# FudanCVL/SynFMC

Measured on AMD Instinct MI355X. Metric: denoising steps/sec, 16x320x512 bf16 U-Net+CMC+OMC, higher is better.
Workload: dtype bf16; 1 GPU; 16x320x512 clip, CFG batch 2, full-width 3D U-Net (1.39B params, random init) + Camera Adapter (CMC) + Object Motion Control (OMC) features, DDIM step; configs/obj.yaml shapes; 1 clip per GPU; frames=16, height=320, width=512, hip_graph=True, fp8_temporal_attention=False, parallelism=dp1 (independent clips, no collective)

## Files before the change

synfmc_amd/csrc/gemm_conv.hip:

```cpp
#include <stdlib.h>

#include <algorithm>
#include <type_traits>

#include "common.h"

namespace {

constexpr int BK_MAX = 64;

struct GemmParams {
    const bf16_t* a; const bf16_t* w; const bf16_t* bias; const bf16_t* temb; const bf16_t* res; bf16_t* out;
    const bf16_t* res2;
    int64_t M; int N, K;
    int64_t lda, ldres, ldo;
    int img_h, img_w, cin, hw;
    int64_t temb_ld; int temb_div;
    const bf16_t* a2; int64_t lda2; int ksplit;
    int ups;
    float alpha;
    int tiles_m, tiles_n;
    int regepi;
    int tap_outer;
    int group_m;
// ... 605 lines not shown
#pragma unroll
                    for (int k = 0; k < 8; ++k) a[k] = (a[k] + ba[k]) * gelu_erf(g[k] + bg[k]);
                    Vec8<bf16_t>::store(P.out + m * P.ldo + no, a);
                }
            }
        }
    }
    if (!SK) break;
    if (sk_partial) {
        asm volatile("s_waitcnt vmcnt(0)" ::: "memory");
        __syncthreads();
        if (tid == 0)
            __hip_atomic_store(P.sk_flags + blockIdx.x, 1, __ATOMIC_RELAXED, __HIP_MEMORY_SCOPE_AGENT);
    } else if (sk_np > 0) {
        __syncthreads();
        if (tid == 0)
            for (int j = 1; j <= sk_np; ++j)
                __hip_atomic_store(P.sk_flags + (blockIdx.x - 8 * j), 0, __ATOMIC_RELAXED, __HIP_MEMORY_SCOPE_AGENT);
    }
    __syncthreads();
    }
}

template <int MODE, int EPI, int PF, int ROLE>
__global__ __launch_bounds__(512, 2)
void gemm8_kernel(const GemmParams P) {
    constexpr int BM = 256, BN = 256, BK = 64, NT = 512;
    constexpr int STAGE_ELEMS = (BM + BN) * BK;
    constexpr int VMW = 2 * (PF - 2);
    static_assert(PF >= 3 && PF <= 6, "prefetch distance (half-tiles)");
    extern __shared__ __attribute__((aligned(16))) unsigned char smem_raw[];
    bf16_t* smem = reinterpret_cast<bf16_t*>(smem_raw);
    const int wave = __builtin_amdgcn_readfirstlane(threadIdx.x >> 6);
    const int wr = wave >> 2, wc = wave & 3;

    const int nkt = P.K / BK;
    constexpr bool SK = ROLE == 1 || ROLE == 3;
    int64_t sk_it = 0, sk_end = 0, sk_gbase = 0, sk_I = 0;
    int sk_r = 0, sk_per = 1, sk_first = 0;
    int lk_u = 0;
    if (SK && P.sk_lock) {
        lk_u = (int)(blockIdx.x & 7) * (P.sk >> 3) + (int)(blockIdx.x >> 3);
    } else if (SK) {
        const int T = P.tiles_m * P.tiles_n - P.sk_t0, x = blockIdx.x & 7, q = blockIdx.x >> 3;
        sk_per = P.sk >> 3;
        const int tg0 = (int)((int64_t)T * x / 8), tg1 = (int)((int64_t)T * (x + 1) / 8);
        sk_gbase = (int64_t)tg0 * nkt;
        sk_I = (int64_t)(tg1 - tg0) * nkt;
        sk_r = sk_per - 1 - q;
// ... 95 lines not shown
#pragma unroll
                        for (int gq = 0; gq < 4; ++gq) {
                            const int quad = (wave * 8 + ni * 4 + mi) * 4 + gq;
                            t[gq] = __builtin_amdgcn_raw_buffer_load_b128(rsP, (int)(((int64_t)slot * (BM * BN / 4) + quad * 64 + lane) * 16), 0, 0);
                        }
#pragma unroll
                        for (int gq = 0; gq < 4; ++gq) {
                            union { u32x4 u; f32x4 f; } c;
                            c.u = t[gq];
                            acc[ni][mi][4 * gq] += c.f[0]; acc[ni][mi][4 * gq + 1] += c.f[1];
                            acc[ni][mi][4 * gq + 2] += c.f[2]; acc[ni][mi][4 * gq + 3] += c.f[3];
                        }
                    }
            }
        }
    }
    const int64_t m0 = (int64_t)tile_m * BM;
    const int n0 = tile_n * BN;

    constexpr unsigned OOB = 0x80000000u;
    const __amdgpu_buffer_rsrc_t rsA = __builtin_amdgcn_make_buffer_rsrc((void*)P.a, 0, (int)P.a_bytes, 0x00020000);
    const __amdgpu_buffer_rsrc_t rsW = __builtin_amdgcn_make_buffer_rsrc((void*)P.w, 0, (int)((int64_t)P.N * P.K * 2), 0x00020000);
    unsigned a_vo[4];
    unsigned a_ok[4];
    unsigned w_vo[4];
    int a_lds[4], w_lds[4];
#pragma unroll
    for (int e = 0; e < 4; ++e) {
        const int late = e >> 1, u = 2 * wave + (e & 1);
        const int rowa = (u >> 3) * 128 + late * 64 + (u & 7) * 8;
        a_lds[e] = rowa * BK;
        const int lr = rowa + prow;
        const int sc = swz<BK>(lr, pch);
        const int64_t m = m0 + lr;
        const bool ok = m < P.M;
        a_ok[e] = 0;
        if (MODE == 0) {
            a_vo[e] = ok ? (unsigned)((m * P.lda + sc * 8) * 2) : OOB;
        } else {
            const int64_t mm = ok ? m : 0;
            const int pix = (int)(mm % P.hw);
            const int py = pix / P.img_w, px = pix - py * P.img_w;
            const int64_t img = mm / P.hw;
            if (P.ups == 1) {
                a_vo[e] = ok ? (unsigned)((img * (int64_t)(P.hw >> 2) * P.cin + sc * 8) * 2) : OOB;
                a_ok[e] = ((unsigned)py << 16) | (unsigned)px;
            } else {
                unsigned mask = 0;
                for (int t = 0; t < 9; ++t) {
                    const int dy = t / 3 - 1, dx = t % 3 - 1;
                    const bool in = P.ups == 2 ? (2 * py + dy >= 0 && 2 * px + dx >= 0)
                                               : ((unsigned)(py + dy) < (unsigned)P.img_h && (unsigned)(px + dx) < (unsigned)P.img_w);
                    mask |= (unsigned)in << t;
                }
                a_ok[e] = ok ? mask : 0u;
                if (P.ups == 2) a_vo[e] = (unsigned)(((img * (int64_t)(P.hw << 2) + (int64_t)(2 * py) * (2 * P.img_w) + 2 * px) * P.cin + sc * 8) * 2);
                else a_vo[e] = (unsigned)((mm * P.cin + sc * 8) * 2);
            }
        }
        const int roww = (u >> 2) * 64 + late * 32 + (u & 3) * 8;
        w_lds[e] = (BM + roww) * BK;
// ... 22 lines not shown
            seek(kt0);
        } else if (MODE == 1) {
            if (P.tap_outer) {
                it_ci0 += BK;
                if (it_ci0 == P.cin) { it_ci0 = 0; ++it_tap; }
            } else if (++it_tap == 9) {
                it_tap = 0;
                it_ci0 += BK;
            }
        }
    };
    auto dma = [&](const __amdgpu_buffer_rsrc_t& rs, unsigned voff, int soff, bf16_t* lds) {
        __builtin_amdgcn_raw_ptr_buffer_load_lds(rs, (__attribute__((address_space(3))) void*)lds, 16, (int)voff, soff, 0, 0);
    };
    auto issue = [&](int q) {
        bf16_t* stage = smem + it_buf * STAGE_ELEMS;
        if (q == 1 || q == 2) {
            const int e0 = (q - 1) * 2;
            const int soff = (MODE == 1 ? it_tap * P.cin + it_ci0 : it_kt * BK) * 2;
#pragma unroll
            for (int i = 0; i < 2; ++i) dma(rsW, w_vo[e0 + i], soff, stage + w_lds[e0 + i]);
        } else {
            const int e0 = q == 0 ? 0 : 2;
            if (MODE == 0) {
#pragma unroll
                for (int i = 0; i < 2; ++i) dma(rsA, a_vo[e0 + i], it_kt * BK * 2, stage + a_lds[e0 + i]);
            } else {
                const int dy = (it_tap >= 3) + (it_tap >= 6) - 1, dx = it_tap - 3 * (dy + 1) - 1;
#pragma unroll
                for (int i = 0; i < 2; ++i) {
                    const int e = e0 + i;
                    unsigned vo;
                    if (P.ups == 1) {
                        const int py = (int)(a_ok[e] >> 16) + dy, px = (int)(a_ok[e] & 0xffffu) + dx;
                        const bool in = (unsigned)py < (unsigned)P.img_h && (unsigned)px < (unsigned)P.img_w;
                        vo = a_vo[e] + (unsigned)(((py >> 1) * (P.img_w >> 1) + (px >> 1)) * P.cin * 2);
                        if (!in || a_vo[e] == OOB) vo = OOB;
                    } else {
                        const int shift = (P.ups == 2 ? (dy * 2 * P.img_w + dx) : (dy * P.img_w + dx)) * P.cin * 2;
                        vo = ((a_ok[e] >> it_tap) & 1u) ? a_vo[e] + (unsigned)shift : OOB;
                    }
                    dma(rsA, vo, it_ci0 * 2, stage + a_lds[e]);
                }
            }
        }
        if (q == 3) advance();
    };
// ... 296 lines not shown
}
__device__ __forceinline__ void gn_tile_finish(const GemmParams& P, float* red, int64_t m0, int n0, int cpg, int tid, float s, float ss) {
    const int GT = 320 / cpg, RP = 512 / GT;
    red[2 * tid] = s;
    red[2 * tid + 1] = ss;
    __syncthreads();
    if (tid < GT) {
        float a = 0.f, b = 0.f;
        for (int k = 0; k < RP; ++k) { a += red[2 * (tid + k * GT)]; b += red[2 * (tid + k * GT) + 1]; }
        const int64_t img = m0 / P.gn_hw;
        const int nsplit = P.gn_hw / 160, sp = (int)((m0 - img * P.gn_hw) / 160);
        float* dst = P.gn_part + ((img * nsplit + sp) * 32 + (n0 / cpg + tid)) * 2;
        dst[0] = a;
        dst[1] = b;
    }
}

__device__ __forceinline__ void lane32_swap(float& lo_keeps, float& hi_keeps) {
    auto r = __builtin_amdgcn_permlane32_swap(__float_as_uint(lo_keeps), __float_as_uint(hi_keeps), false, false);
    lo_keeps = __uint_as_float(r[0]);
    hi_keeps = __uint_as_float(r[1]);
}

template <int MODE, int EPI>
__global__ __launch_bounds__(512, 2)
void gemm160_kernel(const GemmParams P) {
    constexpr int BM = 160, BN = 320, BK = 32, NT = 512, NBUF = 5;
    constexpr int SUB_ELEMS = (BM + BN) * BK;
    extern __shared__ __attribute__((aligned(16))) unsigned char smem_raw[];
    bf16_t* smem = reinterpret_cast<bf16_t*>(smem_raw);
    const int wave = __builtin_amdgcn_readfirstlane(threadIdx.x >> 6);
    const int wr = wave >> 2, wc = wave & 3;
    const int tid = threadIdx.x, lane = tid & 63;
    const int l15 = lane & 15, kq = lane >> 4;
    const int prow = lane >> 2, pch = lane & 3;
    const int psrc = pch ^ (3 * ((prow >> 3) & 1));

    int nks = P.K / BK, ks0 = 0;
    int tile_m, tile_n;
    const int split = P.split_k > 1 ? (int)(blockIdx.x % P.split_k) : 0;
    {
        const int total = P.tiles_m * P.tiles_n;
        int lin = blockIdx.x;
        if (P.split_k > 1) {
            lin = blockIdx.x / P.split_k;
            const int per = ((nks + P.split_k - 1) / P.split_k + 1) & ~1;
            ks0 = split * per;
            nks = max(0, min(nks, ks0 + per) - ks0);
        } else {
            const int id = blockIdx.x, q = total >> 3, r = total & 7, x = id & 7;
            lin = (x < r ? x * (q + 1) : r * (q + 1) + (x - r) * q) + (id >> 3);
        }
        lin_to_tile(lin, P, tile_m, tile_n);
    }
    const int64_t m0 = (int64_t)tile_m * BM;
    const int n0 = tile_n * BN;

    constexpr unsigned OOB = 0x80000000u;
    const __amdgpu_buffer_rsrc_t rsA = __builtin_amdgcn_make_buffer_rsrc((void*)P.a, 0, (int)P.a_bytes, 0x00020000);
    const __amdgpu_buffer_rsrc_t rsW = __builtin_amdgcn_make_buffer_rsrc((void*)P.w, 0, (int)((int64_t)P.N * P.K * 2), 0x00020000);
    unsigned e_vo[4], e_ok[4];
    int e_lds[4];
#pragma unroll
    for (int e = 0; e < 4; ++e) {
        const int i = 4 * wave + e;
        e_vo[e] = OOB; e_ok[e] = 0; e_lds[e] = NBUF * SUB_ELEMS;
        if (i < 20) {
            const int lw = 16 * i + prow, n = n0 + lw;
            e_lds[e] = (BM + 16 * i) * BK;
            e_vo[e] = n >= P.N ? OOB : (P.w_blocked ? (unsigned)((((int64_t)tile_n * (P.K / BK)) * (BN * BK) + lw * BK + psrc * 8) * 2)
                                                     : (unsigned)(((int64_t)n * P.K + psrc * 8) * 2));
        } else if (i < 30) {
            const int lr = 16 * (i - 20) + prow;
            e_lds[e] = 16 * (i - 20) * BK;
            const int64_t m = m0 + lr;
            const bool ok = m < P.M;
            if (MODE == 0) {
                e_vo[e] = ok ? (P.a_blocked ? (unsigned)((((int64_t)tile_m * (P.K / BK)) * (BM * BK) + lr * BK + psrc * 8) * 2)
                                            : (unsigned)((m * P.lda + psrc * 8) * 2)) : OOB;
            } else {
                const int64_t mm = ok ? m : 0;
                const int pix = (int)(mm % P.hw);
                const int py = pix / P.img_w, px = pix - py * P.img_w;
                const int64_t img = mm / P.hw;
                if (P.ups == 1) {
                    e_vo[e] = ok ? (unsigned)((img * (int64_t)(P.hw >> 2) * P.cin + psrc * 8) * 2) : OOB;
                    e_ok[e] = ((unsigned)py << 16) | (unsigned)px;
                } else {
                    unsigned mask = 0;
                    for (int t = 0; t < 9; ++t) {
                        const int dy = t / 3 - 1, dx = t % 3 - 1;
                        const bool in = P.ups == 2 ? (2 * py + dy >= 0 && 2 * px + dx >= 0)
                                                   : ((unsigned)(py + dy) < (unsigned)P.img_h && (unsigned)(px + dx) < (unsigned)P.img_w);
                        mask |= (unsigned)in << t;
                    }
                    e_ok[e] = ok ? mask : 0u;
                    if (P.ups == 2) e_vo[e] = (unsigned)(((img * (int64_t)(P.hw << 2) + (int64_t)(2 * py) * (2 * P.img_w) + 2 * px) * P.cin + psrc * 8) * 2);
                    else e_vo[e] = (unsigned)((mm * P.cin + psrc * 8) * 2);
                }
            }
        }
    }
// ... 13 lines not shown
            seek0();
        } else if (MODE == 1) {
            if (++it_half == 2) {
                it_half = 0;
                if (++it_tap == 9) { it_tap = 0; it_ci0 += 64; }
            }
        }
    };
    auto dma = [&](const __amdgpu_buffer_rsrc_t& rs, unsigned voff, int soff, bf16_t* lds) {
        __builtin_amdgcn_raw_ptr_buffer_load_lds(rs, (__attribute__((address_space(3))) void*)lds, 16, (int)voff, soff, 0, 0);
    };
    auto issue = [&]() {
        bf16_t* stage = smem + it_buf * SUB_ELEMS;
        const int kw = P.w_blocked ? it_s * (BN * BK * 2)
                                   : (MODE == 1 ? it_tap * P.cin + it_ci0 + it_half * 32 : it_s * BK) * 2;
        if (w_wave) {
#pragma unroll
            for (int e = 0; e < 4; ++e) dma(rsW, e_vo[e], kw, stage + e_lds[e]);
        } else {
            const int dy = (it_tap >= 3) + (it_tap >= 6) - 1, dx = it_tap - 3 * (dy + 1) - 1;
#pragma unroll
            for (int e = 0; e < 4; ++e) {
                bf16_t* dst = e_lds[e] == NBUF * SUB_ELEMS ? smem + NBUF * SUB_ELEMS : stage + e_lds[e];
                if (MODE == 0) {
                    dma(rsA, e_vo[e], P.a_blocked ? it_s * (BM * BK * 2) : it_s * BK * 2, dst);
                } else {
                    unsigned vo;
                    if (P.ups == 1) {
                        const int py = (int)(e_ok[e] >> 16) + dy, px = (int)(e_ok[e] & 0xffffu) + dx;
                        const bool in = (unsigned)py < (unsigned)P.img_h && (unsigned)px < (unsigned)P.img_w;
                        vo = e_vo[e] + (unsigned)(((py >> 1) * (P.img_w >> 1) + (px >> 1)) * P.cin * 2);
                        if (!in || e_vo[e] == OOB) vo = OOB;
                    } else {
                        const int shift = (P.ups == 2 ? (dy * 2 * P.img_w + dx) : (dy * P.img_w + dx)) * P.cin * 2;
                        vo = ((e_ok[e] >> it_tap) & 1u) ? e_vo[e] + (unsigned)shift : OOB;
                    }
                    dma(rsA, vo, (it_ci0 + it_half * 32) * 2, dst);
                }
            }
        }
        advance();
    };
    (void)a_first;

    f32x4 acc[5][5];
    bf16x8 wf[5], af[5];
    const int frag_off = l15 * BK + (kq ^ (3 * ((l15 >> 3) & 1))) * 8;
// ... 880 lines not shown
            P.sk_lock_len = L;
            fmc_launch<sk_main>(dim3((unsigned)g), dim3(512), lds, st, P);
            if constexpr (EPI == 0) hipLaunchKernelGGL((sk_finish_kernel<MODE>), dim3((unsigned)tiles * 64), dim3(256), 0, st, P);
            else fmc_launch<sk_finish>(dim3((unsigned)tiles), dim3(512), lds, st, P);
            return;
        }
        P.sk_lock = 0;
    }
    if (P.sk) {
        const int64_t iters = (int64_t)tiles * (P.K / 64);
        const int g = fmc_cu_count() & ~7;
        const int maxseg = (tiles + g - 1) / g + 2;
        const int64_t need = (int64_t)g * maxseg * 256 * 256 * (int64_t)sizeof(float) + 4096;
        if (g >= 8 && iters >= 2 * (int64_t)g && P.sk_ws_bytes >= need && need < ((int64_t)1 << 31)) {
            P.sk = g;
            P.sk_maxseg = maxseg;
            P.sk_whole = 0;
            fmc_launch<sk_main>(dim3((unsigned)g), dim3(512), lds, st, P);
            fmc_launch<sk_finish>(dim3((unsigned)tiles), dim3(512), lds, st, P);
            return;
        }
        P.sk = 0;
    }
    fmc_launch<plain>(dim3((unsigned)tiles), dim3(512), lds, st, P);
}

constexpr int K320_K = 320;
template <int MI, int NI> constexpr int k320_stage_chunks() { return ((32 * MI * ((160 * NI + 8) / 8) + 63) / 64) * 64; }
template <int MI, int NI> constexpr size_t k320_lds() {
    return (size_t)2 * 32 * MI * K320_K * 2 + (size_t)k320_stage_chunks<MI, NI>() * 16 + 160 * NI * sizeof(float);
}

template <int MI, int NI, bool HAS_RES>
__global__ __launch_bounds__(320, (MI * NI == 1 ? 3 : (MI * NI == 2 ? 2 : 1))) void gemm_k320_kernel(const GemmParams P) {
    constexpr int K = K320_K, KS = K / 16, BM = 32 * MI, BN = 160 * NI, OP = BN + 8, CPR = K / 8, OCPR = OP / 8, WC = 32 * NI;
    constexpr int A_ELEMS = BM * K, A_PIECES = BM * CPR / 64, ST_PIECES = k320_stage_chunks<MI, NI>() / 64;
    constexpr int A_PPW = (A_PIECES + 4) / 5, ST_PPW = (ST_PIECES + 4) / 5;
    extern __shared__ __attribute__((aligned(16))) unsigned char smem_raw[];
    bf16_t* Abuf = reinterpret_cast<bf16_t*>(smem_raw);
    bf16_t* Os = Abuf + 2 * A_ELEMS;
    float* bias_s = reinterpret_cast<float*>(Os + k320_stage_chunks<MI, NI>() * 8);
    const int tid = threadIdx.x, lane = tid & 63, wave = __builtin_amdgcn_readfirstlane(tid >> 6);
    const int l31 = lane & 31, half = lane >> 5;
    const int n0 = blockIdx.y * BN;
    const int ntiles = (int)(P.M / BM);

// ... 136 lines not shown
    const int bn = (gemm_k320_cfg() % 10 == 1) ? 160 : 320;
    return !P.f32io && P.hw <= 1 && P.K == K320_K && P.N % bn == 0 && P.M % 64 == 0 && !P.a2 && !P.res2 && P.split_k == 1 && !P.sk && !P.temb &&
           ((P.M - 1) * P.lda + P.K) * 2 < ((int64_t)1 << 31) && (!P.res || ((P.M - 1) * P.ldres + P.N) * 2 < ((int64_t)1 << 31));
}

template <int MI, int NI>
void launch_gemm_k320_c(GemmParams& P, hipStream_t st) {
    const size_t lds = k320_lds<MI, NI>();
    const int per_cu = MI * NI == 1 ? 3 : (MI * NI == 2 ? 2 : 1);
    const int tiles = (int)(P.M / (32 * MI)), slots = fmc_cu_count() * per_cu;
    dim3 grid((unsigned)(tiles < slots ? tiles : slots), (unsigned)(P.N / (160 * NI)));
    if (P.res) fmc_launch<gemm_k320_kernel<MI, NI, true>>(grid, dim3(320), lds, st, P);
    else fmc_launch<gemm_k320_kernel<MI, NI, false>>(grid, dim3(320), lds, st, P);
}
void launch_gemm_k320(GemmParams& P, hipStream_t st) {
    switch (gemm_k320_cfg()) {
        case 11: launch_gemm_k320_c<1, 1>(P, st); break;
        case 21: launch_gemm_k320_c<2, 1>(P, st); break;
        case 12: launch_gemm_k320_c<1, 2>(P, st); break;
        default: launch_gemm_k320_c<2, 2>(P, st); break;
    }
}

bool gemm160_ok(const GemmParams& P) {
    return P.N % 320 == 0 && !P.sk && (!P.a2 || P.a_blocked);
}
template <int MODE, int EPI>
void launch_gemm160(GemmParams& P, hipStream_t st) {
    P.tiles_m = (int)((P.M + 159) / 160);
    P.tiles_n = P.N / 320;
    P.tap_outer = 0;
    P.group_m = xcd_group_m(P, MODE == 0, 32.0, 320, 160);
    constexpr size_t lds = (size_t)5 * (160 + 320) * 32 * sizeof(bf16_t) + 1024;
    static_assert(lds >= (size_t)160 * 328 * 2 && lds >= (size_t)160 * 164 * 4, "epilogue staging fits the operand buffers");
    constexpr auto plain = gemm160_kernel<MODE, EPI>;
    if (P.split_k > 1) {
        if constexpr (EPI == 0) {
            fmc_launch<plain>(dim3((unsigned)(P.tiles_m * P.tiles_n * P.split_k)), dim3(512), lds, st, P);
            const int64_t chunks = P.M * (P.N / 8);
            hipLaunchKernelGGL(splitk_reduce_kernel, dim3((unsigned)((chunks + 255) / 256)), dim3(256), 0, st, P);
        }
        return;
    }
    if constexpr (MODE == 0) {
        const int persist = g160_persist();
        const int cus = fmc_cu_count() & ~7;
        if (persist && !P.f32io && P.M % 160 == 0 && ((persist == 2 || P.a_blocked || P.bias_img) ? P.tiles_m * P.tiles_n >= cus : P.tiles_m * P.tiles_n > cus) && cus >= 8) {
            constexpr size_t ldsp = (size_t)3 * (160 + 320) * 32 * sizeof(bf16_t) + 1024 + (EPI == 1 ? (size_t)160 * 168 * 2 + 4096 : (size_t)80 * 328 * 2 + 5120);
            const bool e0 = EPI == 0;
            const int form = e0 && P.bias_img ? (P.ln_stats ? 5 : 4) : e0 && P.a2 ? 6 : P.lnc_stats ? 1 : e0 && P.ln_out ? 2 : e0 && P.ln_stats ? 3 : 0;
            const dim3 grid((unsigned)cus), block(512);
            if (form == 0) fmc_launch<gemm160p_kernel<EPI, 5>>(grid, block, ldsp, st, P);
            else if (form == 1) fmc_launch<gemm160p_kernel<EPI, 5, 0, 1>>(grid, block, ldsp, st, P);
            if constexpr (EPI == 0) {
                if (form == 2) fmc_launch<gemm160p_kernel<0, 5, 1>>(grid, block, ldsp, st, P);
                else if (form == 3) fmc_launch<gemm160p_kernel<0, 5, 2>>(grid, block, ldsp, st, P);
                else if (form == 4) fmc_launch<gemm160p_kernel<0, 5, 0, 0, 0, 1>>(grid, block, ldsp, st, P);
                else if (form == 5) fmc_launch<gemm160p_kernel<0, 5, 2, 0, 0, 1>>(grid, block, ldsp, st, P);
                else if (form == 6) fmc_launch<gemm160p_kernel<0, 5, 0, 0, 1>>(grid, block, ldsp, st, P);
            }
            return;
        }
    }
    fmc_launch<plain>(dim3((unsigned)(P.tiles_m * P.tiles_n)), dim3(512), lds, st, P);
}

bool gemm256p_ok(const GemmParams& P) {
    const int cus = fmc_cu_count() & ~7;
    return P.N % 320 == 0 && P.M % 256 == 0 && !P.sk && !P.a2 && P.split_k == 1 && !P.f32io && cus >= 8 && (P.M / 256) * (P.N / 320) > cus;
}
void launch_gemm256p(GemmParams& P, hipStream_t st) {
    P.tiles_m = (int)(P.M / 256);
    P.tiles_n = P.N / 320;
    P.tap_outer = 0;
    P.group_m = xcd_group_m(P, true, 32.0, 320, 256);
    constexpr size_t ldsp = (size_t)3 * (256 + 320) * 32 * sizeof(bf16_t) + 1024 + (size_t)128 * 168 * 2;
    static_assert(ldsp <= 160 * 1024, "ring + staging fit the LDS");
    fmc_launch<gemm160p_kernel<1, 8>>(dim3((unsigned)(fmc_cu_count() & ~7)), dim3(512), ldsp, st, P);
}

bool gemm8_ok(GemmParams& P) {
    const int64_t a_elems = P.hw > 1 ? (P.ups == 1 ? (P.M / 4) * (int64_t)P.cin : P.M * (int64_t)P.cin * (P.ups == 2 ? 4 : 1))
                                     : (P.a2 && P.a_blocked ? P.M * (int64_t)P.ksplit : (P.M - 1) * P.lda + P.K);
    P.a_bytes = a_elems * 2;
    return P.split_k == 1 && (!P.a2 || P.a_blocked) && P.a_bytes < ((int64_t)1 << 31) && (int64_t)P.N * P.K * 2 < ((int64_t)1 << 31);
}

constexpr int GEMM_TILE_MAX = 22;

template <int MODE, int EPI>
void launch_gemm(GemmParams& P, int tile, hipStream_t st) {
    int g = gemm_geometry_override();
    if (g == 0) g = tile;
    if (g == 0) {
        auto tiles = [&](int bm, int bn) { return ((P.M + bm - 1) / bm) * ((P.N + bn - 1) / bn); };
        auto waste = [&](int bn) { return (double)(((P.N + bn - 1) / bn) * bn) / P.N; };
        if (tiles(256, 256) >= 256 && waste(256) <= 1.2) g = 3;
        else if (tiles(256, 128) >= 256 && waste(128) <= 1.25) g = 2;
        else g = 1;
    }
    if (g == 17) {
        if constexpr (MODE == 0 && EPI == 1) {
            if (gemm8_ok(P) && gemm256p_ok(P)) { launch_gemm256p(P, st); return; }
        }
        g = 16;
    }
    if (g == 16) {
        const int sk_keep = P.split_k;
        P.split_k = 1;
        const bool fits = gemm8_ok(P);
        P.split_k = sk_keep;
        if (fits && gemm160_ok(P)) { launch_gemm160<MODE, EPI>(P, st); return; }
        g = 13;
    }
    if ((g == 13 || g == 14) && !gemm8_ok(P)) g = 3;
    if (g == 15) {
        if constexpr (MODE == 0 && EPI == 0) {
            if (gemm_k320_ok(P)) { launch_gemm_k320(P, st); return; }
        }
        g = 5;
    }
    if constexpr (MODE == 0 && EPI == 0) {
        if (g >= 19 && g <= 22 && (P.split_k != 1 || P.res2 || P.sk || P.f32io)) g = 1;
        if (g == 19) { launch_gemm_g<0, 0, 2, 2, 64, 3, 1>(P, st); return; }
        if (g == 20) { launch_gemm_g<0, 0, 2, 2, 32, 4, 1>(P, st); return; }
        if (g == 21) { launch_gemm_g<0, 0, 4, 2, 64, 2, 1>(P, st); return; }
        if (g == 22) { launch_gemm_g<0, 0, 2, 4, 64, 2, 1>(P, st); return; }
    }
    switch (g) {
        case 14: launch_gemm8<MODE, EPI, 5>(P, st); break;
        case 13: launch_gemm8<MODE, EPI, 4>(P, st); break;
        case 12: launch_gemm_g<MODE, EPI, 2, 5, 32, 4>(P, st); break;
        case 11: launch_gemm_g<MODE, EPI, 2, 5, 64, 2>(P, st); break;
        case 10: launch_gemm_g<MODE, EPI, 4, 2, 32, 4>(P, st); break;
        case 9: launch_gemm_g<MODE, EPI, 2, 2, 32, 4>(P, st); break;
        case 8: launch_gemm_g<MODE, EPI, 4, 4, 32, 4>(P, st); break;
        case 7: launch_gemm_g<MODE, EPI, 4, 2, 64, 3>(P, st); break;
        case 6: launch_gemm_g<MODE, EPI, 4, 4, 32, 2>(P, st); break;
// ... 364 lines not shown
```

synfmc_amd/hip_ops.py:

```python
from __future__ import annotations

import atexit
import ctypes
import math
import os
from typing import Optional, Tuple

import torch

from . import _lib
from ._lib import FMC_BF16, FMC_F32
from .derived import derived_on_owner

_DT = {torch.bfloat16: FMC_BF16, torch.float32: FMC_F32}


def _dt(t: torch.Tensor) -> int:
    try:
        return _DT[t.dtype]
    except KeyError:
        raise TypeError(f"fmc kernels take bf16 or fp32 activations, got {t.dtype}") from None


def _dev(*ts: torch.Tensor) -> None:
# ... 1393 lines not shown
            tile = 16
        else:
            weight = _w_tilemajor(weight)
    M, ldx = _rows2d(x)
    ldx2, k_split = 0, 0
    if x2 is not None:
        M2, ldx2 = _rows2d(x2)
        k_split = x.shape[-1]
        assert M2 == M and k_split + x2.shape[-1] == Kd
    n_out = N // 2 if geglu else N
    ldo = n_out
    if out is None:
        out = torch.empty(*x.shape[:-1], n_out, dtype=x.dtype, device=x.device)
    else:
        assert out.dtype == x.dtype and out.shape[-1] == n_out and _rows2d(out)[0] == M and tile != 18
        ldo = _rows2d(out)[1]
    ldres = 0
    if residual is not None:
        assert residual.shape == out.shape
        _, ldres = _rows2d(residual)
    if residual2 is not None:
        assert residual is not None and residual2.shape == out.shape and _rows2d(residual2)[1] == ldres
    ws, ws_bytes = _splitk_workspace(x.device, split_k, M, N)
    _log_call("own_linear", (M, N, Kd, "geglu" if geglu else f"t{tile}", (residual is not None) + (residual2 is not None)), 2.0 * M * N * Kd)
    _lib.check(_lib.load().fmc_linear_bf16(x.data_ptr(), weight.data_ptr(), _p(bias), _p(residual), out.data_ptr(), M, N,
                                           Kd, ldx, ldres, ldo, float(alpha), int(geglu), int(tile), int(split_k),
                                           ws, ws_bytes, _p(x2), ldx2, k_split, _p(residual2), _stream()),
               "fmc_linear_bf16")
    return out


def conv3x3_supported(x: torch.Tensor, weight: torch.Tensor, stride, padding) -> bool:
    s2 = tuple(stride) == (2, 2) and x.shape[-1] % 2 == 0 and x.shape[-2] % 2 == 0
    return (x.is_cuda and x.dtype == torch.bfloat16 and weight.dtype == torch.bfloat16
            and tuple(weight.shape[2:]) == (3, 3) and (tuple(stride) == (1, 1) or s2) and tuple(padding) == (1, 1)
            and weight.shape[1] % 64 == 0 and weight.shape[0] % 8 == 0)


def conv3x3_bf16(x_nhwc: torch.Tensor, weight_cl: torch.Tensor, bias: Optional[torch.Tensor] = None,
                 temb: Optional[torch.Tensor] = None, residual_nhwc: Optional[torch.Tensor] = None,
                 tile: int = 0, split_k: int = 1, temb_div: int = 1, upsample: bool = False,
                 stride2: bool = False) -> torch.Tensor:
    _dev(x_nhwc, weight_cl, bias, temb, residual_nhwc)
    n, h, w, cin = x_nhwc.shape
    if upsample:
        h, w = 2 * h, 2 * w
    if stride2:
# ... 286 lines not shown
    M = h.numel() // C
    assert mid_blocked.numel() == M * (Kd - C) and tail_residual.numel() == M * N
    out = torch.empty_like(tail_residual)
    if partial_tiles:
        assert _blocked_storage_ok(mid_blocked, M, Kd - C), "ff_tail: the tile-major operand does not own its padded storage"
        wt = _w_tilemajor(w_cat) if W_TILEMAJOR else w_cat
        _log_call("own_linear", (M, N, Kd, "ff-tail-partial", 1), 2.0 * M * N * Kd)
        _lib.check(_lib.load().fmc_linear_bf16_fftail_partial(mid_blocked.data_ptr(), h.data_ptr(), wt.data_ptr(), _p(b_cat), tail_residual.data_ptr(),
                                                              out.data_ptr(), M, N, Kd, Kd - C, C, N, None, 0, int(W_TILEMAJOR), _stream()),
                   "fmc_linear_bf16_fftail_partial")
        return out
    part = None
    if gn_hw and gn_emit_ok(M, N, Kd, gn_hw, h.dtype):
        part = torch.empty(M // gn_hw, gn_hw // 160, 32, 2, dtype=torch.float32, device=h.device)
        gn_epilogue_calls["emitted"] += 1
    wt = _w_tilemajor(w_cat) if W_TILEMAJOR else w_cat
    _log_call("own_linear", (M, N, Kd, "ff-tail", 1), 2.0 * M * N * Kd)
    _lib.check(_lib.load().fmc_linear_bf16_fftail(mid_blocked.data_ptr(), h.data_ptr(), wt.data_ptr(), _p(b_cat), tail_residual.data_ptr(), out.data_ptr(),
                                                  M, N, Kd, Kd - C, C, N, _p(part), int(gn_hw if part is not None else 0), int(W_TILEMAJOR), _stream()),
               "fmc_linear_bf16_fftail")
    if part is not None:
        out._fmc_gn = (part, N)
    return out


def linear_gn(x: torch.Tensor, weight: torch.Tensor, bias, residual, alpha: float, residual2, hw: int):
    _dev(x, weight, bias, residual)
    N, Kd = weight.shape
    M, ldx = _rows2d(x)
    out = torch.empty(*x.shape[:-1], N, dtype=x.dtype, device=x.device)
    part = torch.empty(M // hw, hw // 160, 32, 2, dtype=torch.float32, device=x.device)
    ldres = 0 if residual is None else _rows2d(residual)[1]
    gn_epilogue_calls["emitted"] += 1
    wt = _w_tilemajor(weight) if W_TILEMAJOR else weight
    _log_call("own_linear", (M, N, Kd, "gn", (residual is not None) + (residual2 is not None)), 2.0 * M * N * Kd)
    _lib.check(_lib.load().fmc_linear_bf16_gn(x.data_ptr(), wt.data_ptr(), _p(bias), _p(residual), out.data_ptr(), M, N, Kd, ldx, ldres, N,
                                              float(alpha), _p(residual2), part.data_ptr(), int(hw), int(W_TILEMAJOR), _stream()), "fmc_linear_bf16_gn")
    out._fmc_gn = (part, N)
    return out


def conv3x3_gn(x_nhwc: torch.Tensor, weight_cl: torch.Tensor, bias, temb, residual_nhwc, temb_div: int, upsample: bool, stride2: bool):
    n, h, w, cin = x_nhwc.shape
    if upsample:
        h, w = 2 * h, 2 * w
    if stride2:
# ... 555 lines not shown
    n320 = (key[5] if key[0] == "conv" else key[2]) % 320 == 0
    cands = tuple(t for t in GEMM_TILES + tuple(extra_arms)
                  if (t != 15 or k320)
                  and (not (ARM_160 <= t < ARM_160 + 5 or ARM_160B <= t < ARM_160B + 5 or t == ARM_256) or n320))
    if use is not None and not (use in cands or (use == 0 and not no_lib) or (use == -1 and key not in _tune_log)):
        _choice.pop(key, None)
        _tune_log.pop(key, None)
        stale_table_entries[0] += 1
        use = None
    if use is None:
        if not AUTOTUNE or torch.cuda.is_current_stream_capturing():
            return 0 if not (static_hip or no_lib) else -1
        times = ([] if no_lib else [(_time_ms(lib_fn), 0)]) + [(_time_ms(lambda t=t: hip_fn(t)), t) for t in cands]
        use = min(times)[1]
        _choice[key] = use
        _tune_log[key] = {arm: round(ms, 4) for ms, arm in times}
        _cache_state["dirty"] = True
    return use


def linear(x: torch.Tensor, weight: torch.Tensor, bias: Optional[torch.Tensor] = None,
           residual: Optional[torch.Tensor] = None, alpha: float = 1.0, x2: Optional[torch.Tensor] = None,
           residual2: Optional[torch.Tensor] = None, gn_hw: int = 0, ln: Optional["LnSpec"] = None,
           lazy_residual: bool = False) -> torch.Tensor:
    import torch.nn.functional as F
    pend = getattr(x, "_fmc_pending_ln", None)
    if pend is not None:
        if (x2 is None and residual is None and residual2 is None and alpha == 1.0 and not gn_hw and ln is None and weight.is_contiguous()
                and lnc_ok(x, weight)):
            dispatch_calls["linear"]["own"] += 1
            return linear_lnc(x, weight, bias, pend)
        x = resolve_pending_ln(x)

    def lib():
        xin = x if x2 is None else torch.cat([x, x2], dim=-1)
        if alpha == 1.0 and vendor_linear_ok(xin, weight, bias, residual):
            y = vendor_linear(xin, weight, bias, residual)
            return y if residual2 is None else y + residual2
        y = F.linear(xin, weight, bias)
        _log_call("vendor", (xin.numel() // xin.shape[-1], weight.shape[0], weight.shape[1], bias is not None, False), 2.0 * xin.numel() * weight.shape[0])
        if residual is not None:
            y = torch.add(residual, y, alpha=alpha)
            return y if residual2 is None else y + residual2
        return y if alpha == 1.0 else y * alpha

    N, Kd = weight.shape
    if (F32_GEMM and x.is_cuda and x.dtype == torch.float32 and weight.dtype == torch.float32 and Kd % 64 == 0 and N % 8 == 0
# ... 11 lines not shown
        dispatch_calls["linear"]["ineligible"] += 1
        return lib()
    M = x.numel() // x.shape[-1]
    if ln is not None and x2 is None and not gn_hw and ln_emit_ok(x, weight, residual, residual2, ln):
        dispatch_calls["linear"]["own"] += 1
        return linear_ln(x, weight, bias, residual, alpha, residual2, ln)
    if (gn_hw and x2 is None and x.is_contiguous() and gn_emit_ok(M, N, Kd, gn_hw, x.dtype)
            and (residual is None or (residual.is_contiguous() and residual.dtype == x.dtype))
            and (residual2 is None or residual2.is_contiguous())):
        dispatch_calls["linear"]["own"] += 1
        return linear_gn(x, weight, bias, residual, alpha, residual2, gn_hw)
    key = ("lin", M, N, Kd, bias is not None, (residual is not None) + (residual2 is not None),
           0 if x2 is None else x.shape[-1])
    hip = lambda tile: (linear4_bf16(x, weight, bias, residual, alpha, residual2) if tile == ARM_G4
                        else linear_bf16(x, weight, bias, residual, alpha, tile=tile, x2=x2, residual2=residual2))
    small = (ARM_SMALLM, ARM_SMALLM + 2) if (M <= 2560 and x2 is None and residual2 is None) else ()
    t160 = ((M + 159) // 160) * ((N + 159) // 160)
    if (LINEAR4 and x2 is None and weight.is_contiguous() and 48 <= t160 <= 640 and Kd >= 320
            and _lib.load().fmc_linear4_supported(M, N, Kd, _rows2d(x)[1])
            and (residual is None or _rows2d(residual)[1] % 8 == 0)
            and (residual2 is None or (residual is not None and _rows2d(residual2)[1] == _rows2d(residual)[1]))):
        small = small + (ARM_G4,)
    use = _pick(key, hip, lib, Kd <= 640 and N <= 1024 and M >= 16384, split_arms(M, N, Kd) + small,
                k320=(Kd == 320 and N % 320 == 0 and M % 64 == 0 and x2 is None and residual2 is None))
    if (use == 0 and lazy_residual and LAZY_RESIDUAL and residual is not None and residual2 is None and alpha == 1.0 and x2 is None
            and N in (320, 640, 1280) and residual.is_contiguous() and not torch.is_grad_enabled()
            and not vendor_linear_ok(x, weight, bias, residual)):
        dispatch_calls["linear"]["vendor"] += 1
        y = F.linear(x, weight, bias)
        y._fmc_pending_add = residual
        return y
    dispatch_calls["linear"]["vendor" if use == 0 else "own"] += 1
    return lib() if use == 0 else hip(max(use, 0))


def geglu_linear(x: torch.Tensor, weight: torch.Tensor, bias, weight_il: torch.Tensor, bias_il, weight_il160=None,
                 bias_il160=None) -> torch.Tensor:
    import torch.nn.functional as F
    pend = getattr(x, "_fmc_pending_ln", None)
    if pend is not None:
        if weight_il160 is not None and weight_il160.is_contiguous() and lnc_ok(x, weight_il160):
            return linear_lnc(x, weight_il160, bias_il160, pend, geglu=True)
        x = resolve_pending_ln(x)
    lib = lambda: geglu(F.linear(x, weight, bias))
    if (F32_GEMM and x.is_cuda and x.dtype == torch.float32 and weight_il.dtype == torch.float32 and weight_il.shape[0] % 64 == 0
            and weight_il.shape[1] % 64 == 0 and x.is_contiguous()):
        N, Kd = weight.shape
# ... 781 lines not shown
```

synfmc_amd/models/layers.py:

```python
from __future__ import annotations

import os

import math
from typing import Optional

import torch
import torch.nn.functional as F
from torch import nn

from .. import hip_ops as K
from ..derived import derived, drop


def to_tokens(x: torch.Tensor) -> torch.Tensor:
    n, c, h, w = x.shape
    t = x.permute(0, 2, 3, 1)
    if not t.is_contiguous():
        t = t.contiguous()
    return K.carry_gn(x, t.view(n, h * w, c))


def from_tokens(t: torch.Tensor, h: int, w: int) -> torch.Tensor:
    n, _, c = t.shape
# ... 706 lines not shown
        pending = getattr(h, "_fmc_pending_add", None) is not None or getattr(h, "_fmc_ln", None) is not None \
            or getattr(h, "_fmc_pending_ln", None) is not None
        if not pending and self.ln_partial_route(h):
            return self._forward_ln_partial(h, norm, residual, tail)
        if not K.geglu_ln_direct_ok(h, w) or pending:
            return None
        M = h.numel() // h.shape[-1]
        pipe = K.geglu_ln_pipe_ok(h, w) and (h.shape[-1] == 320 or K.GEGLU_PIPE_640)
        var = K.geglu_pipe_variant(M, h.shape[-1]) if pipe else -1
        frag = derived(self, "_geglu_frag", [w], lambda: K.pack_geglu_frag(w, 16 if var == 1 else 32) if pipe else K.pack_geglu_frag80(w), extra=(var,))
        blocked = K.geglu_direct_blocked_ok(h, out.weight, residual)
        if pipe:
            mid = K.geglu_ln_pipe(h, f32_param(norm, "weight"), f32_param(norm, "bias"), norm.eps, frag, proj.proj.bias, w.shape[0] // 2, blocked=blocked,
                                  variant=var)
        else:
            mid = K.geglu_ln_direct(h, f32_param(norm, "weight"), f32_param(norm, "bias"), norm.eps, frag, proj.proj.bias, w.shape[0] // 2, blocked=blocked)
        if blocked and tail is not None and residual is h and K.ff_tail_ok(h, out.weight, tail[0], tail[2]):
            wc, bc = self._tail_weights(tail[0], tail[1])
            y = K.ff_tail(mid, h, wc, bc, tail[2], tail[3])
            y._fmc_tail = True
            return y
        if blocked:
            return K.linear_from_blocked(mid, out.weight, out.bias, residual)
        return out(mid, residual=residual)

    def forward(self, hidden_states, scale: float = 1.0, residual: Optional[torch.Tensor] = None):
        proj, out = self.net[0], self.net[2]
        if not torch.is_grad_enabled() and own_trainable(out, hidden_states):
            return shadow_twin(self)(hidden_states, residual=residual)
        il = proj.interleaved() if (hidden_states.is_cuda and hidden_states.dtype == torch.bfloat16 and not torch.is_grad_enabled()) else None
        if il is not None and K.ff_blocked_ok(hidden_states, il[2], out.weight, residual):
            mid = K.geglu_linear_blocked(hidden_states, il[2], il[3])
            return K.linear_from_blocked(mid, out.weight, out.bias, residual)
        return out(proj(hidden_states), residual=residual)


class BasicTransformerBlock(nn.Module):
    def __init__(self, dim, num_attention_heads, attention_head_dim, dropout=0.0, cross_attention_dim=None,
                 activation_fn="geglu", attention_bias=False, only_cross_attention=False,
                 double_self_attention=False, upcast_attention=False, norm_elementwise_affine=True,
                 norm_type="layer_norm", norm_eps=1e-5, final_dropout=False):
        super().__init__()
        assert norm_type == "layer_norm" and not only_cross_attention and not double_self_attention
        self.norm1 = LayerNorm(dim, elementwise_affine=norm_elementwise_affine, eps=norm_eps)
        self.attn1 = Attention(query_dim=dim, heads=num_attention_heads, dim_head=attention_head_dim, dropout=dropout,
                               bias=attention_bias, upcast_attention=upcast_attention)
# ... 163 lines not shown
```

Baseline: 41.64 steps/s.

## Fuse FF output and tail projection via row-major second-A GEMM segment

Adds a second row-major A operand to the gemm8 and gemm160 token-mode kernels. Past a K split point they load from a separate tensor, so a GEMM can read the concatenation [mid | h] without building it in memory. The feed-forward path for C=640 row-major (non-blocked) layers uses this to fold the FF output projection and the following tail projection into one GEMM with concatenated weights. This removes an intermediate write/read and a launch. In exchange, persistent gemm160 is disabled for this case, and the new kernel template variants add code size.

```diff
diff --git a/synfmc_amd/csrc/gemm_conv.hip b/synfmc_amd/csrc/gemm_conv.hip
--- a/synfmc_amd/csrc/gemm_conv.hip
+++ b/synfmc_amd/csrc/gemm_conv.hip
@@ -651,9 +651,10 @@
     }
 }
 
-template <int MODE, int EPI, int PF, int ROLE>
+template <int MODE, int EPI, int PF, int ROLE, int A2 = 0>
 __global__ __launch_bounds__(512, 2)
 void gemm8_kernel(const GemmParams P) {
+    static_assert(!A2 || (MODE == 0 && ROLE == 0), "the second A segment exists in token mode on the plain grid");
     constexpr int BM = 256, BN = 256, BK = 64, NT = 512;
     constexpr int STAGE_ELEMS = (BM + BN) * BK;
     constexpr int VMW = 2 * (PF - 2);
@@ -795,6 +796,8 @@
     const __amdgpu_buffer_rsrc_t rsA = __builtin_amdgcn_make_buffer_rsrc((void*)P.a, 0, (int)P.a_bytes, 0x00020000);
     const __amdgpu_buffer_rsrc_t rsW = __builtin_amdgcn_make_buffer_rsrc((void*)P.w, 0, (int)((int64_t)P.N * P.K * 2), 0x00020000);
     unsigned a_vo[4];
+    const __amdgpu_buffer_rsrc_t rsA2 = __builtin_amdgcn_make_buffer_rsrc((void*)(A2 ? P.a2 : P.a), 0, A2 ? (int)(((P.M - 1) * P.lda2 + (P.K - P.ksplit)) * 2) : 0, 0x00020000);
+    unsigned a_vo2[4];
     unsigned a_ok[4];
     unsigned w_vo[4];
     int a_lds[4], w_lds[4];
@@ -810,6 +813,7 @@
         a_ok[e] = 0;
         if (MODE == 0) {
             a_vo[e] = ok ? (unsigned)((m * P.lda + sc * 8) * 2) : OOB;
+            if (A2) a_vo2[e] = ok ? (unsigned)((m * P.lda2 + sc * 8) * 2) : OOB;
         } else {
             const int64_t mm = ok ? m : 0;
             const int pix = (int)(mm % P.hw);
@@ -878,7 +882,10 @@
             for (int i = 0; i < 2; ++i) dma(rsW, w_vo[e0 + i], soff, stage + w_lds[e0 + i]);
         } else {
             const int e0 = q == 0 ? 0 : 2;
-            if (MODE == 0) {
+            if (A2 && it_kt * BK >= P.ksplit) {
+#pragma unroll
+                for (int i = 0; i < 2; ++i) dma(rsA2, a_vo2[e0 + i], (it_kt * BK - P.ksplit) * 2, stage + a_lds[e0 + i]);
+            } else if (MODE == 0) {
 #pragma unroll
                 for (int i = 0; i < 2; ++i) dma(rsA, a_vo[e0 + i], it_kt * BK * 2, stage + a_lds[e0 + i]);
             } else {
@@ -1221,9 +1228,10 @@
     hi_keeps = __uint_as_float(r[1]);
 }
 
-template <int MODE, int EPI>
+template <int MODE, int EPI, int A2 = 0>
 __global__ __launch_bounds__(512, 2)
 void gemm160_kernel(const GemmParams P) {
+    static_assert(!A2 || MODE == 0, "the second A segment exists in token mode");
     constexpr int BM = 160, BN = 320, BK = 32, NT = 512, NBUF = 5;
     constexpr int SUB_ELEMS = (BM + BN) * BK;
     extern __shared__ __attribute__((aligned(16))) unsigned char smem_raw[];
@@ -1258,12 +1266,14 @@
     constexpr unsigned OOB = 0x80000000u;
     const __amdgpu_buffer_rsrc_t rsA = __builtin_amdgcn_make_buffer_rsrc((void*)P.a, 0, (int)P.a_bytes, 0x00020000);
     const __amdgpu_buffer_rsrc_t rsW = __builtin_amdgcn_make_buffer_rsrc((void*)P.w, 0, (int)((int64_t)P.N * P.K * 2), 0x00020000);
-    unsigned e_vo[4], e_ok[4];
+    const __amdgpu_buffer_rsrc_t rsA2 = __builtin_amdgcn_make_buffer_rsrc((void*)(A2 ? P.a2 : P.a), 0, A2 ? (int)(((P.M - 1) * P.lda2 + (P.K - P.ksplit)) * 2) : 0, 0x00020000);
+    unsigned e_vo[4], e_ok[4], e_vo2[4];
     int e_lds[4];
 #pragma unroll
     for (int e = 0; e < 4; ++e) {
         const int i = 4 * wave + e;
         e_vo[e] = OOB; e_ok[e] = 0; e_lds[e] = NBUF * SUB_ELEMS;
+        if (A2) e_vo2[e] = OOB;
         if (i < 20) {
             const int lw = 16 * i + prow, n = n0 + lw;
             e_lds[e] = (BM + 16 * i) * BK;
@@ -1277,6 +1287,7 @@
             if (MODE == 0) {
                 e_vo[e] = ok ? (P.a_blocked ? (unsigned)((((int64_t)tile_m * (P.K / BK)) * (BM * BK) + lr * BK + psrc * 8) * 2)
                                             : (unsigned)((m * P.lda + psrc * 8) * 2)) : OOB;
+                if (A2) e_vo2[e] = ok ? (unsigned)((m * P.lda2 + psrc * 8) * 2) : OOB;
             } else {
                 const int64_t mm = ok ? m : 0;
                 const int pix = (int)(mm % P.hw);
@@ -1336,7 +1347,9 @@
 #pragma unroll
             for (int e = 0; e < 4; ++e) {
                 bf16_t* dst = e_lds[e] == NBUF * SUB_ELEMS ? smem + NBUF * SUB_ELEMS : stage + e_lds[e];
-                if (MODE == 0) {
+                if (A2 && it_s * BK >= P.ksplit) {
+                    dma(rsA2, e_vo2[e], (it_s * BK - P.ksplit) * 2, dst);
+                } else if (MODE == 0) {
                     dma(rsA, e_vo[e], P.a_blocked ? it_s * (BM * BK * 2) : it_s * BK * 2, dst);
                 } else {
                     unsigned vo;
@@ -2263,6 +2276,12 @@
         }
         P.sk = 0;
     }
+    if constexpr (MODE == 0 && EPI == 0) {
+        if (P.a2 && !P.a_blocked) {
+            fmc_launch<gemm8_kernel<0, 0, PF, 0, 1>>(dim3((unsigned)tiles), dim3(512), lds, st, P);
+            return;
+        }
+    }
     fmc_launch<plain>(dim3((unsigned)tiles), dim3(512), lds, st, P);
 }
 
@@ -2445,8 +2464,13 @@
     }
 }
 
+bool a2_rowmajor_ok(const GemmParams& P, int ktile) {
+    return P.a2 && !P.a_blocked && P.hw <= 1 && !P.f32io && P.split_k == 1 && !P.sk && P.ksplit > 0 && P.ksplit < P.K && P.ksplit % ktile == 0 &&
+           ((P.M - 1) * P.lda2 + (P.K - P.ksplit)) * 2 < ((int64_t)1 << 31);
+}
+
 bool gemm160_ok(const GemmParams& P) {
-    return P.N % 320 == 0 && !P.sk && (!P.a2 || P.a_blocked);
+    return P.N % 320 == 0 && !P.sk && (!P.a2 || P.a_blocked || (a2_rowmajor_ok(P, 32) && !P.w_blocked));
 }
 template <int MODE, int EPI>
 void launch_gemm160(GemmParams& P, hipStream_t st) {
@@ -2468,7 +2492,7 @@
     if constexpr (MODE == 0) {
         const int persist = g160_persist();
         const int cus = fmc_cu_count() & ~7;
-        if (persist && !P.f32io && P.M % 160 == 0 && ((persist == 2 || P.a_blocked || P.bias_img) ? P.tiles_m * P.tiles_n >= cus : P.tiles_m * P.tiles_n > cus) && cus >= 8) {
+        if (persist && !(P.a2 && !P.a_blocked) && !P.f32io && P.M % 160 == 0 && ((persist == 2 || P.a_blocked || P.bias_img) ? P.tiles_m * P.tiles_n >= cus : P.tiles_m * P.tiles_n > cus) && cus >= 8) {
             constexpr size_t ldsp = (size_t)3 * (160 + 320) * 32 * sizeof(bf16_t) + 1024 + (EPI == 1 ? (size_t)160 * 168 * 2 + 4096 : (size_t)80 * 328 * 2 + 5120);
             const bool e0 = EPI == 0;
             const int form = e0 && P.bias_img ? (P.ln_stats ? 5 : 4) : e0 && P.a2 ? 6 : P.lnc_stats ? 1 : e0 && P.ln_out ? 2 : e0 && P.ln_stats ? 3 : 0;
@@ -2485,6 +2509,12 @@
             return;
         }
     }
+    if constexpr (MODE == 0 && EPI == 0) {
+        if (P.a2 && !P.a_blocked) {
+            fmc_launch<gemm160_kernel<0, 0, 1>>(dim3((unsigned)(P.tiles_m * P.tiles_n)), dim3(512), lds, st, P);
+            return;
+        }
+    }
     fmc_launch<plain>(dim3((unsigned)(P.tiles_m * P.tiles_n)), dim3(512), lds, st, P);
 }
 
@@ -2504,9 +2534,9 @@
 
 bool gemm8_ok(GemmParams& P) {
     const int64_t a_elems = P.hw > 1 ? (P.ups == 1 ? (P.M / 4) * (int64_t)P.cin : P.M * (int64_t)P.cin * (P.ups == 2 ? 4 : 1))
-                                     : (P.a2 && P.a_blocked ? P.M * (int64_t)P.ksplit : (P.M - 1) * P.lda + P.K);
+                                     : (P.a2 && P.a_blocked ? P.M * (int64_t)P.ksplit : (P.M - 1) * P.lda + (P.a2 ? P.ksplit : P.K));
     P.a_bytes = a_elems * 2;
-    return P.split_k == 1 && (!P.a2 || P.a_blocked) && P.a_bytes < ((int64_t)1 << 31) && (int64_t)P.N * P.K * 2 < ((int64_t)1 << 31);
+    return P.split_k == 1 && (!P.a2 || P.a_blocked || a2_rowmajor_ok(P, 64)) && P.a_bytes < ((int64_t)1 << 31) && (int64_t)P.N * P.K * 2 < ((int64_t)1 << 31);
 }
 
 constexpr int GEMM_TILE_MAX = 22;
@@ -2522,6 +2552,7 @@
         else if (tiles(256, 128) >= 256 && waste(128) <= 1.25) g = 2;
         else g = 1;
     }
+    const bool a2rm = P.a2 && !P.a_blocked;
     if (g == 17) {
         if constexpr (MODE == 0 && EPI == 1) {
             if (gemm8_ok(P) && gemm256p_ok(P)) { launch_gemm256p(P, st); return; }
@@ -2533,10 +2564,10 @@
         P.split_k = 1;
         const bool fits = gemm8_ok(P);
         P.split_k = sk_keep;
-        if (fits && gemm160_ok(P)) { launch_gemm160<MODE, EPI>(P, st); return; }
+        if (fits && gemm160_ok(P) && (!a2rm || (MODE == 0 && EPI == 0))) { launch_gemm160<MODE, EPI>(P, st); return; }
         g = 13;
     }
-    if ((g == 13 || g == 14) && !gemm8_ok(P)) g = 3;
+    if ((g == 13 || g == 14) && (!gemm8_ok(P) || (a2rm && !(MODE == 0 && EPI == 0)))) g = 3;
     if (g == 15) {
         if constexpr (MODE == 0 && EPI == 0) {
             if (gemm_k320_ok(P)) { launch_gemm_k320(P, st); return; }
diff --git a/synfmc_amd/hip_ops.py b/synfmc_amd/hip_ops.py
--- a/synfmc_amd/hip_ops.py
+++ b/synfmc_amd/hip_ops.py
@@ -1439,7 +1439,8 @@
     if residual2 is not None:
         assert residual is not None and residual2.shape == out.shape and _rows2d(residual2)[1] == ldres
     ws, ws_bytes = _splitk_workspace(x.device, split_k, M, N)
-    _log_call("own_linear", (M, N, Kd, "geglu" if geglu else f"t{tile}", (residual is not None) + (residual2 is not None)), 2.0 * M * N * Kd)
+    _log_call("own_linear", (M, N, Kd, ("geglu" if geglu else f"t{tile}") + ("+x2" if x2 is not None else ""), (residual is not None) + (residual2 is not None)),
+              2.0 * M * N * Kd)
     _lib.check(_lib.load().fmc_linear_bf16(x.data_ptr(), weight.data_ptr(), _p(bias), _p(residual), out.data_ptr(), M, N,
                                            Kd, ldx, ldres, ldo, float(alpha), int(geglu), int(tile), int(split_k),
                                            ws, ws_bytes, _p(x2), ldx2, k_split, _p(residual2), _stream()),
@@ -1772,6 +1773,27 @@
     if part is not None:
         out._fmc_gn = (part, N)
     return out
+
+
+FF_TAIL_L1 = FF_TAIL and os.environ.get("FMC_FF_TAIL_L1", "1") != "0"
+
+
+def ff_tail_rowmajor_ok(h: torch.Tensor, w2: torch.Tensor, wp: torch.Tensor, tail_residual: Optional[torch.Tensor], gn_hw: int = 0) -> bool:
+    C = h.shape[-1]
+    M = h.numel() // C
+    return (FF_TAIL_L1 and not torch.is_grad_enabled() and C == 640 and h.dtype == torch.bfloat16 and h.is_contiguous()
+            and wp.dtype == torch.bfloat16 and w2.dtype == torch.bfloat16 and wp.ndim == 2 and wp.shape[1] == w2.shape[0] == C and wp.shape[0] % 8 == 0
+            and w2.shape[1] % 64 == 0 and tail_residual is not None and tail_residual.dtype == h.dtype and tail_residual.is_contiguous()
+            and tail_residual.numel() == M * wp.shape[0] and not (gn_hw and gn_emit_ok(M, wp.shape[0], w2.shape[1] + C, gn_hw, h.dtype)))
+
+
+def ff_tail_rowmajor(mid: torch.Tensor, h: torch.Tensor, w_cat: torch.Tensor, b_cat: Optional[torch.Tensor], tail_residual: torch.Tensor) -> torch.Tensor:
+    N, Kd = w_cat.shape
+    C = h.shape[-1]
+    M = h.numel() // C
+    assert mid.is_contiguous() and mid.numel() == M * (Kd - C) and tail_residual.numel() == M * N
+    y = linear(mid.view(M, Kd - C), w_cat, b_cat, tail_residual.view(M, N), x2=h.view(M, C), own_only=True)
+    return y.view(tail_residual.shape)
 
 
 def linear_gn(x: torch.Tensor, weight: torch.Tensor, bias, residual, alpha: float, residual2, hw: int):
@@ -2373,7 +2395,7 @@
 def linear(x: torch.Tensor, weight: torch.Tensor, bias: Optional[torch.Tensor] = None,
            residual: Optional[torch.Tensor] = None, alpha: float = 1.0, x2: Optional[torch.Tensor] = None,
            residual2: Optional[torch.Tensor] = None, gn_hw: int = 0, ln: Optional["LnSpec"] = None,
-           lazy_residual: bool = False) -> torch.Tensor:
+           lazy_residual: bool = False, own_only: bool = False) -> torch.Tensor:
     import torch.nn.functional as F
     pend = getattr(x, "_fmc_pending_ln", None)
     if pend is not None:
@@ -2431,7 +2453,7 @@
             and (residual2 is None or (residual is not None and _rows2d(residual2)[1] == _rows2d(residual)[1]))):
         small = small + (ARM_G4,)
     use = _pick(key, hip, lib, Kd <= 640 and N <= 1024 and M >= 16384, split_arms(M, N, Kd) + small,
-                k320=(Kd == 320 and N % 320 == 0 and M % 64 == 0 and x2 is None and residual2 is None))
+                k320=(Kd == 320 and N % 320 == 0 and M % 64 == 0 and x2 is None and residual2 is None), own_only=own_only)
     if (use == 0 and lazy_residual and LAZY_RESIDUAL and residual is not None and residual2 is None and alpha == 1.0 and x2 is None
             and N in (320, 640, 1280) and residual.is_contiguous() and not torch.is_grad_enabled()
             and not vendor_linear_ok(x, weight, bias, residual)):
diff --git a/synfmc_amd/models/layers.py b/synfmc_amd/models/layers.py
--- a/synfmc_amd/models/layers.py
+++ b/synfmc_amd/models/layers.py
@@ -752,6 +752,11 @@
             return y
         if blocked:
             return K.linear_from_blocked(mid, out.weight, out.bias, residual)
+        if tail is not None and residual is h and K.ff_tail_rowmajor_ok(h, out.weight, tail[0], tail[2], tail[3]):
+            wc, bc = self._tail_weights(tail[0], tail[1])
+            y = K.ff_tail_rowmajor(mid, h, wc, bc, tail[2])
+            y._fmc_tail = True
+            return y
         return out(mid, residual=residual)
 
     def forward(self, hidden_states, scale: float = 1.0, residual: Optional[torch.Tensor] = None):
```

After: 41.94 steps/s, median of 6. About the same (+0.7%).
